# anovos/anovos

Measured on AMD Instinct MI355X. Metric: rows/sec (whole node) full analyzer+drift+transform, higher is better.
Workload: dtype fp32 data + fp64 accumulators; 1 GPU; model=anovos-full-pipeline, rows_per_gpu=125000000, n_cols=201, global_batch=125000000, parallelism=dp1

## Files before the change

### anovos_amd/ops/hip/corr_mfma.hip

```cpp

#include <hip/hip_runtime.h>
#include <cfloat>
#include <cstdint>
#include <cmath>

#define THREADS 256

using bf16x8 = __attribute__((ext_vector_type(8))) short;
using f32x4 = __attribute__((ext_vector_type(4))) float;

__device__ __forceinline__ short to_bf16(float v) {
  union {
    float f;
    uint32_t u;
  } c{v};
  uint32_t r = c.u + 0x7FFFu + ((c.u >> 16) & 1u);
  return (short)(r >> 16);
}

__device__ __forceinline__ bf16x8 load_frag(const float *const *cols, int k,
                                            const float *means, int col,
                                            int64_t row, int64_t limit) {
  bf16x8 f;
  if (col < k) {
    const float *__restrict__ x = cols[col];
    const float m = means[col];
    if (row + 8 <= limit) {
      const float4 *p = reinterpret_cast<const float4 *>(x + row);
      float4 a = p[0], b = p[1];
      float v0 = a.x - m, v1 = a.y - m, v2 = a.z - m, v3 = a.w - m;
      float v4 = b.x - m, v5 = b.y - m, v6 = b.z - m, v7 = b.w - m;
      f[0] = to_bf16(isnan(v0) ? 0.f : v0);
      f[1] = to_bf16(isnan(v1) ? 0.f : v1);
      f[2] = to_bf16(isnan(v2) ? 0.f : v2);
      f[3] = to_bf16(isnan(v3) ? 0.f : v3);
      f[4] = to_bf16(isnan(v4) ? 0.f : v4);
      f[5] = to_bf16(isnan(v5) ? 0.f : v5);
      f[6] = to_bf16(isnan(v6) ? 0.f : v6);
      f[7] = to_bf16(isnan(v7) ? 0.f : v7);
    } else {
#pragma unroll
      for (int e = 0; e < 8; ++e) {
        float v = (row + e < limit) ? x[row + e] - m : 0.f;
        f[e] = to_bf16(isnan(v) ? 0.f : v);
      }
    }
  } else {
#pragma unroll
    for (int e = 0; e < 8; ++e) f[e] = 0;
  }
  return f;
}

__global__ __launch_bounds__(THREADS) void gram_partials_kernel(
    const float *const *cols, int64_t n, int k, const float *means,
    const int *pair_i, const int *pair_j, int row_chunks, float *partials) {
  const int pair = blockIdx.x / row_chunks;
  const int chunk = blockIdx.x % row_chunks;
  const int i0 = pair_i[pair] * 16;
  const int j0 = pair_j[pair] * 16;

  const int64_t steps_total = (n + 31) / 32;
  const int64_t steps_per = (steps_total + row_chunks - 1) / row_chunks;
  const int64_t step_s = (int64_t)chunk * steps_per;
  const int64_t step_e = min(steps_total, step_s + steps_per);

  const int lane = threadIdx.x & 63;
  const int wave = threadIdx.x >> 6;
  const int m = lane & 15;
  const int ko = (lane >> 4) * 8;

  f32x4 acc = {0.f, 0.f, 0.f, 0.f};
  for (int64_t s = step_s + wave; s < step_e; s += 4) {
    const int64_t r = s * 32 + ko;
    bf16x8 a = load_frag(cols, k, means, i0 + m, r, n);
    bf16x8 b = (j0 == i0) ? a : load_frag(cols, k, means, j0 + m, r, n);
    acc = __builtin_amdgcn_mfma_f32_16x16x32_bf16(a, b, acc, 0, 0, 0);
  }

  __shared__ float lds[4][256];
#pragma unroll
  for (int reg = 0; reg < 4; ++reg) {
    const int row = (lane >> 4) * 4 + reg;
    lds[wave][row * 16 + (lane & 15)] = acc[reg];
  }
  __syncthreads();
  const int c = threadIdx.x;
  partials[(int64_t)blockIdx.x * 256 + c] =
      lds[0][c] + lds[1][c] + lds[2][c] + lds[3][c];
}

__global__ __launch_bounds__(THREADS) void gram_reduce_kernel(
    const float *partials, int row_chunks, const int *pair_i,
    const int *pair_j, int k, float *gram) {
  const int pair = blockIdx.x;
  const int c = threadIdx.x;
  const int row = c >> 4, col = c & 15;
  double s = 0.0;
  for (int ch = 0; ch < row_chunks; ++ch)
    s += (double)partials[((int64_t)pair * row_chunks + ch) * 256 + c];
  const int gi = pair_i[pair] * 16 + row;
  const int gj = pair_j[pair] * 16 + col;
  if (gi < k && gj < k) {
    gram[(int64_t)gi * k + gj] = (float)s;
    gram[(int64_t)gj * k + gi] = (float)s;
  }
}

extern "C" int anovos_centered_gram(const void *const *cols, int64_t n, int k,
                                    const float *means, const int *pair_i,
                                    const int *pair_j, int npairs,
                                    int row_chunks, float *partials,
                                    float *gram, hipStream_t stream) {
  dim3 grid1((uint32_t)(npairs * row_chunks));
  hipLaunchKernelGGL(gram_partials_kernel, grid1, dim3(THREADS), 0, stream,
                     (const float *const *)cols, n, k, means, pair_i, pair_j,
                     row_chunks, partials);
  hipLaunchKernelGGL(gram_reduce_kernel, dim3((uint32_t)npairs), dim3(THREADS),
                     0, stream, partials, row_chunks, pair_i, pair_j, k, gram);
  return (int)hipGetLastError();
}


typedef short bf16x4_t __attribute__((ext_vector_type(4)));
typedef float nat_f4c __attribute__((ext_vector_type(4)));

template <int MAXPW>
__global__ __launch_bounds__(THREADS) void gram_singleread_kernel(
    const float *const *cols, int64_t n, int k, int ktot, const float *means,
    const int *pair_i, const int *pair_j, int npairs, int row_chunks,
    float *partials) {
  constexpr int STAGES = 4;
  const int kstride = ktot + 3;
  extern __shared__ short slab[];
  const int block = blockIdx.x;
  const int64_t macro_total = (n + STAGES * 32 - 1) / (STAGES * 32);
  const int64_t macro_per = (macro_total + row_chunks - 1) / row_chunks;
  const int64_t mac_s = (int64_t)block * macro_per;
  const int64_t mac_e = min(macro_total, mac_s + macro_per);

  const int lane = threadIdx.x & 63;
  const int wave = threadIdx.x >> 6;
  const int m = lane & 15;
  const int kog = lane >> 4;

  const int ppw = (npairs + 3) / 4;
  const int p0 = wave * ppw;
  int i0s[MAXPW], j0s[MAXPW];
#pragma unroll
  for (int u = 0; u < MAXPW; ++u) {
    const int p = p0 + u;
    const bool act = (u < ppw) && (p < npairs);
    i0s[u] = act ? pair_i[p] * 16 : -1;
    j0s[u] = act ? pair_j[p] * 16 : 0;
  }
  f32x4 acc[MAXPW];
#pragma unroll
  for (int u = 0; u < MAXPW; ++u) acc[u] = f32x4{0.f, 0.f, 0.f, 0.f};

  for (int64_t s = mac_s; s < mac_e; ++s) {
    const int64_t r0 = s * (STAGES * 32);
    __syncthreads();
    for (int idx = threadIdx.x; idx < ktot * 8 * STAGES; idx += THREADS) {
      const int c = idx >> (3 + 2);
      const int seg = idx & (8 * STAGES - 1);
      const int64_t r = r0 + (int64_t)seg * 4;
      float v0 = 0.f, v1 = 0.f, v2 = 0.f, v3 = 0.f;
      if (c < k) {
        const float *__restrict__ x = cols[c];
        const float mean = means[c];
        if (r + 4 <= n) {
          const nat_f4c t = __builtin_nontemporal_load(
              reinterpret_cast<const nat_f4c *>(x + r));
          v0 = t.x - mean; v1 = t.y - mean; v2 = t.z - mean; v3 = t.w - mean;
        } else {
          v0 = (r + 0 < n) ? x[r + 0] - mean : 0.f;
          v1 = (r + 1 < n) ? x[r + 1] - mean : 0.f;
          v2 = (r + 2 < n) ? x[r + 2] - mean : 0.f;
          v3 = (r + 3 < n) ? x[r + 3] - mean : 0.f;
        }
      }
      bf16x4_t pack;
      pack.x = to_bf16(isnan(v0) ? 0.f : v0);
      pack.y = to_bf16(isnan(v1) ? 0.f : v1);
      pack.z = to_bf16(isnan(v2) ? 0.f : v2);
      pack.w = to_bf16(isnan(v3) ? 0.f : v3);
      const int st = seg >> 3;
      const int si = seg & 7;
      short *dst = slab + ((size_t)(st * 4 + (si >> 1)) * kstride + c) * 8 +
                   (size_t)(si & 1) * 4;
      *reinterpret_cast<bf16x4_t *>(dst) = pack;
    }
    __syncthreads();
#pragma unroll
    for (int st = 0; st < STAGES; ++st) {
      const short *sbase = slab + (size_t)st * 4 * kstride * 8;
#pragma unroll
      for (int u = 0; u < MAXPW; ++u) {
        if (i0s[u] >= 0) {
          const bf16x8 a = *reinterpret_cast<const bf16x8 *>(
              sbase + ((size_t)kog * kstride + i0s[u] + m) * 8);
          const bf16x8 b = *reinterpret_cast<const bf16x8 *>(
              sbase + ((size_t)kog * kstride + j0s[u] + m) * 8);
          acc[u] = __builtin_amdgcn_mfma_f32_16x16x32_bf16(a, b, acc[u], 0, 0, 0);
        }
      }
    }
  }

  const int row = (lane >> 4) * 4;
#pragma unroll
  for (int u = 0; u < MAXPW; ++u) {
    const int p = p0 + u;
    if (u < ppw && p < npairs) {
#pragma unroll
      for (int reg = 0; reg < 4; ++reg)
        partials[((int64_t)block * npairs + p) * 256 + (row + reg) * 16 + m] =
            acc[u][reg];
    }
  }
}

__global__ __launch_bounds__(THREADS) void gram_reduce_sr_kernel(
    const float *partials, int nblocks, int npairs, const int *pair_i,
    const int *pair_j, int k, float *gram) {
  const int pair = blockIdx.x;
  const int c = threadIdx.x;
  double s = 0.0;
  for (int ch = 0; ch < nblocks; ++ch)
    s += (double)partials[((int64_t)ch * npairs + pair) * 256 + c];
  const int row = c >> 4, col = c & 15;
  const int gi = pair_i[pair] * 16 + row;
  const int gj = pair_j[pair] * 16 + col;
  if (gi < k && gj < k) {
    gram[(int64_t)gi * k + gj] = (float)s;
    gram[(int64_t)gj * k + gi] = (float)s;
  }
}

extern "C" int anovos_centered_gram_sr(const void *const *cols, int64_t n,
                                       int k, const float *means,
                                       const int *pair_i, const int *pair_j,
                                       int npairs, int row_chunks,
                                       float *partials, float *gram,
                                       hipStream_t stream) {
  const int kt = (k + 15) / 16;
  const int ktot = kt * 16;
  const size_t lds = (size_t)4  * 4 * (ktot + 3) * 16;
  if (kt <= 10)
    hipLaunchKernelGGL((gram_singleread_kernel<14>), dim3(row_chunks),
                       dim3(THREADS), lds, stream, (const float *const *)cols,
                       n, k, ktot, means, pair_i, pair_j, npairs, row_chunks,
                       partials);
  else if (kt <= 13)
    hipLaunchKernelGGL((gram_singleread_kernel<23>), dim3(row_chunks),
                       dim3(THREADS), lds, stream, (const float *const *)cols,
                       n, k, ktot, means, pair_i, pair_j, npairs, row_chunks,
                       partials);
  else
    return -2;
  hipLaunchKernelGGL(gram_reduce_sr_kernel, dim3((uint32_t)npairs),
                     dim3(THREADS), 0, stream, partials, row_chunks, npairs,
                     pair_i, pair_j, k, gram);
  return (int)hipGetLastError();
}

extern "C" int anovos_gram_sr_grid(int k) {
  const int kt = (k + 15) / 16;
  const int ktot = kt * 16;
  const size_t lds = (size_t)4 * 4 * (ktot + 3) * 16;
  static int cached_k = -1, cached_grid = 0;
  if (k == cached_k) return cached_grid;
  int per_cu = 0;
  using KFn = void (*)(const float *const *, int64_t, int, int, const float *,
                       const int *, const int *, int, int, float *);
  KFn fn = (kt <= 10) ? (KFn)gram_singleread_kernel<14>
                      : (KFn)gram_singleread_kernel<23>;
  (void)hipOccupancyMaxActiveBlocksPerMultiprocessor(
      &per_cu, reinterpret_cast<const void *>(fn), THREADS, lds);
  if (per_cu <= 0) per_cu = 3;
  hipDeviceProp_t prop;
  int dev = 0;
  hipGetDevice(&dev);
  hipGetDeviceProperties(&prop, dev);
  int grid = per_cu * (prop.multiProcessorCount > 0 ? prop.multiProcessorCount : 256);
  cached_k = k;
  cached_grid = grid;
  return grid;
}
```

Measured before the change: 404.8 million rows/sec.

## Specialize gram kernel per tile count and prefetch next macro-block loads

The single-read centered Gram kernel is now templated on the exact number of 16-column tiles. That gives compile-time pair counts, static LDS, cached means in shared memory and precomputed per-thread column pointers. Full row blocks run a software-pipelined loop that issues global loads for the next block before the MFMA phase of the current one, with a separate tail path for the partial block. This targets load latency and the index arithmetic of the old generic loop, at the cost of higher register pressure (launch bounds set to 2 blocks) and 13 template instantiations.

```diff
diff --git a/anovos_amd/ops/hip/corr_mfma.hip b/anovos_amd/ops/hip/corr_mfma.hip
--- a/anovos_amd/ops/hip/corr_mfma.hip
+++ b/anovos_amd/ops/hip/corr_mfma.hip
@@ -124,98 +124,178 @@
 
 typedef short bf16x4_t __attribute__((ext_vector_type(4)));
 typedef float nat_f4c __attribute__((ext_vector_type(4)));
-
-template <int MAXPW>
-__global__ __launch_bounds__(THREADS) void gram_singleread_kernel(
-    const float *const *cols, int64_t n, int k, int ktot, const float *means,
+typedef const float __attribute__((address_space(1))) *gcolptr;
+typedef const nat_f4c __attribute__((address_space(1))) *gvecptr;
+
+__device__ __forceinline__ bf16x4_t pack_bf16x4(float v0, float v1, float v2,
+                                                float v3) {
+  bf16x4_t pack;
+  pack.x = to_bf16(isnan(v0) ? 0.f : v0);
+  pack.y = to_bf16(isnan(v1) ? 0.f : v1);
+  pack.z = to_bf16(isnan(v2) ? 0.f : v2);
+  pack.w = to_bf16(isnan(v3) ? 0.f : v3);
+  return pack;
+}
+
+template <int KT>
+__global__ __launch_bounds__(THREADS, 2) void gram_singleread_kernel(
+    const float *const *cols, int64_t n, int k, const float *means,
     const int *pair_i, const int *pair_j, int npairs, int row_chunks,
     float *partials) {
   constexpr int STAGES = 4;
-  const int kstride = ktot + 3;
-  extern __shared__ short slab[];
+  constexpr int KTOT = KT * 16;
+  constexpr int NIT = KTOT / 8;
+  constexpr int PPW = (KT * (KT + 1) / 2 + 3) / 4;
+  constexpr bool PREFETCH = KT <= 10;
+  constexpr int NB = 8;
+  constexpr int KSTRIDE = KTOT + 3;
+  __shared__ __attribute__((aligned(16))) short slab[STAGES * 4 * KSTRIDE * 8];
+  __shared__ float smean[KTOT];
+  __shared__ gcolptr sptr[PREFETCH ? 1 : KTOT];
+
   const int block = blockIdx.x;
   const int64_t macro_total = (n + STAGES * 32 - 1) / (STAGES * 32);
   const int64_t macro_per = (macro_total + row_chunks - 1) / row_chunks;
   const int64_t mac_s = (int64_t)block * macro_per;
   const int64_t mac_e = min(macro_total, mac_s + macro_per);
+  const int64_t full_e = min(mac_e, n / (STAGES * 32));
 
   const int lane = threadIdx.x & 63;
   const int wave = threadIdx.x >> 6;
   const int m = lane & 15;
   const int kog = lane >> 4;
 
-  const int ppw = (npairs + 3) / 4;
-  const int p0 = wave * ppw;
-  int i0s[MAXPW], j0s[MAXPW];
-#pragma unroll
-  for (int u = 0; u < MAXPW; ++u) {
-    const int p = p0 + u;
-    const bool act = (u < ppw) && (p < npairs);
-    i0s[u] = act ? pair_i[p] * 16 : -1;
-    j0s[u] = act ? pair_j[p] * 16 : 0;
-  }
-  f32x4 acc[MAXPW];
-#pragma unroll
-  for (int u = 0; u < MAXPW; ++u) acc[u] = f32x4{0.f, 0.f, 0.f, 0.f};
-
-  for (int64_t s = mac_s; s < mac_e; ++s) {
-    const int64_t r0 = s * (STAGES * 32);
+  const int cw = threadIdx.x >> 5;
+  const int seg = threadIdx.x & 31;
+  const int sst = seg >> 3;
+  const int ssi = seg & 7;
+  short *const dst0 =
+      slab + ((sst * 4 + (ssi >> 1)) * KSTRIDE + cw) * 8 + (ssi & 1) * 4;
+  int kfull = k >> 3;
+  const bool part = cw < (k & 7);
+  gcolptr xp[NIT];
+#pragma unroll
+  for (int it = 0; it < NIT; ++it) {
+    const int c = cw + 8 * it;
+    if (PREFETCH) xp[it] = (gcolptr)cols[min(c, k - 1)] + seg * 4;
+    if (c >= k)
+      *reinterpret_cast<bf16x4_t *>(dst0 + it * 64) = bf16x4_t{0, 0, 0, 0};
+  }
+  if (!PREFETCH)
+    for (int c = threadIdx.x; c < KTOT; c += THREADS)
+      sptr[c] = (gcolptr)cols[min(c, k - 1)];
+  const int cpart = cw + 8 * kfull;
+  const gcolptr xpart = (gcolptr)cols[min(cpart, k - 1)] + seg * 4;
+  short *const dpart = dst0 + kfull * 64;
+  for (int c = threadIdx.x; c < KTOT; c += THREADS)
+    smean[c] = (c < k) ? means[c] : 0.f;
+
+  const int p0 = wave * PPW;
+  int i0s[PPW], j0s[PPW];
+#pragma unroll
+  for (int u = 0; u < PPW; ++u) {
+    const int p = (p0 + u < npairs) ? p0 + u : 0;
+    i0s[u] = __builtin_amdgcn_readfirstlane(pair_i[p] * 16);
+    j0s[u] = __builtin_amdgcn_readfirstlane(pair_j[p] * 16);
+  }
+  f32x4 acc[PPW];
+#pragma unroll
+  for (int u = 0; u < PPW; ++u) acc[u] = f32x4{0.f, 0.f, 0.f, 0.f};
+
+  nat_f4c pre[NIT], prepart;
+  auto issue = [&](int b0, int b1, int64_t off) {
+    if (b0 == 0 && part)
+      prepart = __builtin_nontemporal_load((gvecptr)(xpart + off));
+#pragma unroll
+    for (int it = b0; it < b1; ++it)
+      if (it < kfull) {
+        const gcolptr x = PREFETCH ? xp[it] : sptr[cw + 8 * it] + seg * 4;
+        pre[it] = __builtin_nontemporal_load((gvecptr)(x + off));
+      }
+  };
+  auto stage = [&](const nat_f4c t, float mean, short *dst) {
+    *reinterpret_cast<bf16x4_t *>(dst) =
+        pack_bf16x4(t.x - mean, t.y - mean, t.z - mean, t.w - mean);
+  };
+  auto convert = [&](int b0, int b1) {
+    if (b0 == 0 && part) stage(prepart, smean[cpart], dpart);
+    float mean = smean[cw + 8 * b0];
+#pragma unroll
+    for (int it = b0; it < b1; ++it)
+      if (it < kfull) {
+        const float mnext = smean[cw + 8 * (it + 1 < b1 ? it + 1 : it)];
+        stage(pre[it], mean, dst0 + it * 64);
+        mean = mnext;
+      }
+    __builtin_amdgcn_s_waitcnt(0x0F70);
+  };
+  auto mfma_phase = [&]() {
+#pragma unroll
+    for (int st = 0; st < STAGES; ++st) {
+      const short *sbase = slab + ((st * 4 + kog) * KSTRIDE + m) * 8;
+#pragma unroll
+      for (int u = 0; u < PPW; ++u) {
+        const bf16x8 a = *reinterpret_cast<const bf16x8 *>(sbase + i0s[u] * 8);
+        const bf16x8 b = *reinterpret_cast<const bf16x8 *>(sbase + j0s[u] * 8);
+        acc[u] = __builtin_amdgcn_mfma_f32_16x16x32_bf16(a, b, acc[u], 0, 0, 0);
+      }
+    }
+  };
+  if (PREFETCH && mac_s < full_e) issue(0, NIT, mac_s * (STAGES * 32));
+  for (int64_t s = mac_s; s < full_e; ++s) {
+    asm volatile("" : "+s"(kfull));
     __syncthreads();
-    for (int idx = threadIdx.x; idx < ktot * 8 * STAGES; idx += THREADS) {
-      const int c = idx >> (3 + 2);
-      const int seg = idx & (8 * STAGES - 1);
-      const int64_t r = r0 + (int64_t)seg * 4;
-      float v0 = 0.f, v1 = 0.f, v2 = 0.f, v3 = 0.f;
+    if (PREFETCH) {
+      convert(0, NIT);
+    } else {
+#pragma unroll
+      for (int b = 0; b < NIT; b += NB) {
+        issue(b, b + NB < NIT ? b + NB : NIT, s * (STAGES * 32));
+        convert(b, b + NB < NIT ? b + NB : NIT);
+      }
+    }
+    __syncthreads();
+    if (PREFETCH && s + 1 < full_e) issue(0, NIT, (s + 1) * (STAGES * 32));
+    mfma_phase();
+  }
+
+  if (mac_s < mac_e && full_e < mac_e) {
+    const int64_t r = full_e * (STAGES * 32) + (int64_t)seg * 4;
+    __syncthreads();
+#pragma unroll 1
+    for (int it = 0; it < NIT; ++it) {
+      const int c = cw + 8 * it;
       if (c < k) {
-        const float *__restrict__ x = cols[c];
-        const float mean = means[c];
+        const gcolptr x = (gcolptr)cols[c] + r;
+        const float mean = smean[c];
+        float v0, v1, v2, v3;
         if (r + 4 <= n) {
-          const nat_f4c t = __builtin_nontemporal_load(
-              reinterpret_cast<const nat_f4c *>(x + r));
+          const nat_f4c t = __builtin_nontemporal_load((gvecptr)x);
           v0 = t.x - mean; v1 = t.y - mean; v2 = t.z - mean; v3 = t.w - mean;
         } else {
-          v0 = (r + 0 < n) ? x[r + 0] - mean : 0.f;
-          v1 = (r + 1 < n) ? x[r + 1] - mean : 0.f;
-          v2 = (r + 2 < n) ? x[r + 2] - mean : 0.f;
-          v3 = (r + 3 < n) ? x[r + 3] - mean : 0.f;
+          v0 = (r + 0 < n) ? x[0] - mean : 0.f;
+          v1 = (r + 1 < n) ? x[1] - mean : 0.f;
+          v2 = (r + 2 < n) ? x[2] - mean : 0.f;
+          v3 = (r + 3 < n) ? x[3] - mean : 0.f;
         }
-      }
-      bf16x4_t pack;
-      pack.x = to_bf16(isnan(v0) ? 0.f : v0);
-      pack.y = to_bf16(isnan(v1) ? 0.f : v1);
-      pack.z = to_bf16(isnan(v2) ? 0.f : v2);
-      pack.w = to_bf16(isnan(v3) ? 0.f : v3);
-      const int st = seg >> 3;
-      const int si = seg & 7;
-      short *dst = slab + ((size_t)(st * 4 + (si >> 1)) * kstride + c) * 8 +
-                   (size_t)(si & 1) * 4;
-      *reinterpret_cast<bf16x4_t *>(dst) = pack;
+        *reinterpret_cast<bf16x4_t *>(dst0 + it * 64) =
+            pack_bf16x4(v0, v1, v2, v3);
+      }
     }
     __syncthreads();
-#pragma unroll
-    for (int st = 0; st < STAGES; ++st) {
-      const short *sbase = slab + (size_t)st * 4 * kstride * 8;
-#pragma unroll
-      for (int u = 0; u < MAXPW; ++u) {
-        if (i0s[u] >= 0) {
-          const bf16x8 a = *reinterpret_cast<const bf16x8 *>(
-              sbase + ((size_t)kog * kstride + i0s[u] + m) * 8);
-          const bf16x8 b = *reinterpret_cast<const bf16x8 *>(
-              sbase + ((size_t)kog * kstride + j0s[u] + m) * 8);
-          acc[u] = __builtin_amdgcn_mfma_f32_16x16x32_bf16(a, b, acc[u], 0, 0, 0);
-        }
-      }
-    }
+    mfma_phase();
   }
 
   const int row = (lane >> 4) * 4;
-#pragma unroll
-  for (int u = 0; u < MAXPW; ++u) {
+  int np = npairs;
+  asm volatile("" : "+s"(np));
+#pragma unroll
+  for (int u = 0; u < PPW; ++u) {
     const int p = p0 + u;
-    if (u < ppw && p < npairs) {
+    if (p < np) {
 #pragma unroll
       for (int reg = 0; reg < 4; ++reg)
-        partials[((int64_t)block * npairs + p) * 256 + (row + reg) * 16 + m] =
+        partials[((int64_t)block * np + p) * 256 + (row + reg) * 16 + m] =
             acc[u][reg];
     }
   }
@@ -238,27 +318,39 @@
   }
 }
 
+using SrKernel = void (*)(const float *const *, int64_t, int, const float *,
+                          const int *, const int *, int, int, float *);
+
+static SrKernel gram_sr_instance(int kt) {
+  switch (kt) {
+    case 1: return gram_singleread_kernel<1>;
+    case 2: return gram_singleread_kernel<2>;
+    case 3: return gram_singleread_kernel<3>;
+    case 4: return gram_singleread_kernel<4>;
+    case 5: return gram_singleread_kernel<5>;
+    case 6: return gram_singleread_kernel<6>;
+    case 7: return gram_singleread_kernel<7>;
+    case 8: return gram_singleread_kernel<8>;
+    case 9: return gram_singleread_kernel<9>;
+    case 10: return gram_singleread_kernel<10>;
+    case 11: return gram_singleread_kernel<11>;
+    case 12: return gram_singleread_kernel<12>;
+    case 13: return gram_singleread_kernel<13>;
+    default: return nullptr;
+  }
+}
+
 extern "C" int anovos_centered_gram_sr(const void *const *cols, int64_t n,
                                        int k, const float *means,
                                        const int *pair_i, const int *pair_j,
                                        int npairs, int row_chunks,
                                        float *partials, float *gram,
                                        hipStream_t stream) {
-  const int kt = (k + 15) / 16;
-  const int ktot = kt * 16;
-  const size_t lds = (size_t)4  * 4 * (ktot + 3) * 16;
-  if (kt <= 10)
-    hipLaunchKernelGGL((gram_singleread_kernel<14>), dim3(row_chunks),
-                       dim3(THREADS), lds, stream, (const float *const *)cols,
-                       n, k, ktot, means, pair_i, pair_j, npairs, row_chunks,
-                       partials);
-  else if (kt <= 13)
-    hipLaunchKernelGGL((gram_singleread_kernel<23>), dim3(row_chunks),
-                       dim3(THREADS), lds, stream, (const float *const *)cols,
-                       n, k, ktot, means, pair_i, pair_j, npairs, row_chunks,
-                       partials);
-  else
-    return -2;
+  const SrKernel fn = gram_sr_instance((k + 15) / 16);
+  if (!fn) return -2;
+  hipLaunchKernelGGL(fn, dim3(row_chunks), dim3(THREADS), 0, stream,
+                     (const float *const *)cols, n, k, means, pair_i, pair_j,
+                     npairs, row_chunks, partials);
   hipLaunchKernelGGL(gram_reduce_sr_kernel, dim3((uint32_t)npairs),
                      dim3(THREADS), 0, stream, partials, row_chunks, npairs,
                      pair_i, pair_j, k, gram);
@@ -266,19 +358,14 @@
 }
 
 extern "C" int anovos_gram_sr_grid(int k) {
-  const int kt = (k + 15) / 16;
-  const int ktot = kt * 16;
-  const size_t lds = (size_t)4 * 4 * (ktot + 3) * 16;
   static int cached_k = -1, cached_grid = 0;
   if (k == cached_k) return cached_grid;
+  const SrKernel fn = gram_sr_instance((k + 15) / 16);
   int per_cu = 0;
-  using KFn = void (*)(const float *const *, int64_t, int, int, const float *,
-                       const int *, const int *, int, int, float *);
-  KFn fn = (kt <= 10) ? (KFn)gram_singleread_kernel<14>
-                      : (KFn)gram_singleread_kernel<23>;
-  (void)hipOccupancyMaxActiveBlocksPerMultiprocessor(
-      &per_cu, reinterpret_cast<const void *>(fn), THREADS, lds);
-  if (per_cu <= 0) per_cu = 3;
+  if (fn)
+    (void)hipOccupancyMaxActiveBlocksPerMultiprocessor(
+        &per_cu, reinterpret_cast<const void *>(fn), THREADS, 0);
+  if (per_cu <= 0) per_cu = 2;
   hipDeviceProp_t prop;
   int dev = 0;
   hipGetDevice(&dev);
```

New measurement: 431.6 million rows/sec (median of 6 runs). +6.6%, better.
